# ihmcrobotics/mecano

Hardware: AMD Instinct MI355X
Metric: robot-configs/sec (RNEA+ABA), 30-DoF humanoid batch=4096 (higher is better)
Workload: dtype f64; 1 GPU; 30-DoF humanoid (SixDoF pelvis + 24 revolute), RNEA and ABA of every configuration per step, fp64, AoS [B][n] state; entry_point=mh_rnea_aba_f64, batch_per_gpu=4096, global_batch=4096, nq=31, nv=30, bodies=25, parallelism=dp1 (batch sharded, no data-path collective), kernel_variant=topo:b5c1e26c784c54fa, model_seed=43, state_seed=2342

## Files before the change

mecano_amd/csrc/mh_zv_kernels.h:

```cpp
#pragma once
#include "mh_spec_kernels.h"

namespace mh
{
template <class TP>
struct ZvStore
{
   static constexpr int REG_SLOTS = Split<TP>::zv_reg_slots();
   static constexpr int kind(int j) { return Split<TP>::is_trunk(j) ? ST_LDS_KIND : ST_REG_KIND; }
   static constexpr int index(int j) { return Split<TP>::is_trunk(j) ? Split<TP>::zv_trunk_slot(j) : Split<TP>::zv_reg_slot(j); }
   static constexpr bool shared(int j) { return !Split<TP>::is_trunk(j); }
};
template <class TP>
struct ZvbStore
{
   using S = Split<TP>;
   static constexpr bool root_in_regs(int j) { return S::staged() && j == S::root(); }
   static constexpr int REG_SLOTS = S::zv_reg_slots() + (S::staged() ? Tree<TP>::zv_slots_of(S::root() < 0 ? 0 : S::root(), true) : 0);
   static constexpr int trunk_slot(int j)
   {
      int s = 0;
      for (int i = 0; i < j; i++)
         s += S::is_trunk(i) && !root_in_regs(i) ? Tree<TP>::zv_slots_of(i, false) : 0;
      return s;
   }
   static constexpr int TRUNK_SLOTS = trunk_slot(TP::N);
   static constexpr int kind(int j) { return S::is_trunk(j) && !root_in_regs(j) ? ST_LDS_KIND : ST_REG_KIND; }
   static constexpr int index(int j) { return root_in_regs(j) ? S::zv_reg_slots() : (S::is_trunk(j) ? trunk_slot(j) : S::zv_reg_slot(j)); }
   static constexpr bool shared(int j) { return kind(j) == ST_REG_KIND; }
};
template <class TP>
struct ZvfPlan;
template <class TP>
struct ZvfStore
{
   using S = Split<TP>;
   using TR = Tree<TP>;
   static constexpr bool slot_homes = true;
   static constexpr bool mailed(int j) { return ZvfPlan<TP>::use_mail() && !S::is_trunk(j) && S::limb_index_of_body(j) == S::mailed_limb(); }
   static constexpr int slot_kind(int j, int k) { return mailed(j) && k >= 7 ? ST_LDS_KIND : kind(j); }
   static constexpr int slot_index(int j, int k) { return mailed(j) && k >= 7 ? ZvfPlan<TP>::mail_base() + (k - 7) : index(j) + k; }
   static constexpr bool root_in_regs(int j) { return S::staged() && j == S::root(); }
   static constexpr int limb_slots(int j) { return TR::zv_slots_of(j, true) + TR::ndof(j); }
   static constexpr int reg_slot(int j)
   {
      int s = 0;
      for (int i = 0; i < j; i++)
         s += !S::is_trunk(i) && S::owner(S::limb_index_of_body(i)) == S::owner(S::limb_index_of_body(j)) ? limb_slots(i) : 0;
      return s;
   }
   static constexpr int limb_reg_slots()
   {
      int best = 0;
      for (int w = 0; w < 4; w++)
      {
         int n = 0;
         for (int j = 0; j < TP::N; j++)
            n += !S::is_trunk(j) && S::owner(S::limb_index_of_body(j)) == w ? limb_slots(j) : 0;
         best = n > best ? n : best;
      }
      return best;
   }
   static constexpr int REG_SLOTS = limb_reg_slots() + (S::staged() ? TR::zv_slots_of(S::root() < 0 ? 0 : S::root(), true) : 0);
   static constexpr int trunk_slot(int j)
   {
      int s = 0;
      for (int i = 0; i < j; i++)
         s += S::is_trunk(i) && !root_in_regs(i) ? TR::zv_slots_of(i, false) + TR::ndof(i) : 0;
      return s;
   }
   static constexpr int root_tau_slot() { return trunk_slot(TP::N); }
   static constexpr int ROOT_TAU_SLOTS = S::staged() ? TR::ndof(S::root() < 0 ? 0 : S::root()) : 0;
   static constexpr bool owns_late(int w)
   {
      for (int k = 0; k < S::n_limbs(); k++)
         if (S::is_late(k) && S::owner(k) == w)
            return true;
      return false;
   }
   static constexpr bool late_body(int j) { return S::staged() && !S::is_trunk(j) && owns_late(S::owner(S::limb_index_of_body(j))); }
   static constexpr int late_tau_slot(int j)
   {
      int s = trunk_slot(TP::N) + ROOT_TAU_SLOTS;
      for (int i = 0; i < j; i++)
         s += late_body(i) ? TR::ndof(i) : 0;
      return s;
   }
   static constexpr int TRUNK_SLOTS = late_tau_slot(TP::N);
   static constexpr int tau_slot(int j) { return TR::zv_slots_of(j, !S::is_trunk(j)); }
   static constexpr int kind(int j) { return S::is_trunk(j) && !root_in_regs(j) ? ST_LDS_KIND : ST_REG_KIND; }
   static constexpr int index(int j) { return root_in_regs(j) ? limb_reg_slots() : (S::is_trunk(j) ? trunk_slot(j) : reg_slot(j)); }
   static constexpr bool shared(int j) { return kind(j) == ST_REG_KIND; }
};
#ifdef MH_ZV_PROBE
__device__ unsigned long long zv_probe[4096 * 3 * 4 * 16];
#define ZV_STAMP(job, ph)                                                                                                                  \
   do                                                                                                                                      \
   {                                                                                                                                       \
      const unsigned long long t_ = __builtin_amdgcn_s_memrealtime();                                                                      \
      if ((threadIdx.x & 63) == 0 && k < 4096)                                                                                             \
         zv_probe[((k * 3 + (job)) * 4 + (threadIdx.x >> 6)) * 16 + (ph)] = t_;                                                            \
   } while (0)
__device__ unsigned long long zv_probe_body[4096 * 32 * 4];
#ifdef MH_ZV_PROBE_BODY
#define ZV_STAMP_BODY(body, ph)                                                                                                            \
   do                                                                                                                                      \
   {                                                                                                                                       \
      const unsigned long long t_ = __builtin_amdgcn_s_memrealtime();                                                                      \
      if ((threadIdx.x & 63) == 0 && cx.own < 4096 && ((body) != 0 || cx.wave == 0))                                                      \
         zv_probe_body[(cx.own * 32 + (body)) * 4 + (ph)] = t_;                                                                            \
   } while (0)
#else
#define ZV_STAMP_BODY(body, ph)
#endif
#else
#define ZV_STAMP(job, ph)
#define ZV_STAMP_BODY(body, ph)
#endif
MH_DEV void zv_lds_barrier()
{
   asm volatile("s_waitcnt lgkmcnt(0)\n\ts_barrier" ::: "memory");
}
template <class CX>
MH_DEV void zv_fold_barrier()
{
   zv_lds_barrier();
}
constexpr int ZV_XW = 21;

template <int LIMB, class CX, typename T>
MH_DEV void x_put_ia(const CX &cx, const ABI<T> &I)
{
   constexpr int XW = ZV_XW;
   x_put<LIMB, XW, 0, CX, T>(cx, I.A.xx), x_put<LIMB, XW, 1, CX, T>(cx, I.A.xy), x_put<LIMB, XW, 2, CX, T>(cx, I.A.xz);
   x_put<LIMB, XW, 3, CX, T>(cx, I.A.yy), x_put<LIMB, XW, 4, CX, T>(cx, I.A.yz), x_put<LIMB, XW, 5, CX, T>(cx, I.A.zz);
   x_put<LIMB, XW, 6, CX, T>(cx, I.L.xx), x_put<LIMB, XW, 7, CX, T>(cx, I.L.xy), x_put<LIMB, XW, 8, CX, T>(cx, I.L.xz);
   x_put<LIMB, XW, 9, CX, T>(cx, I.L.yy), x_put<LIMB, XW, 10, CX, T>(cx, I.L.yz), x_put<LIMB, XW, 11, CX, T>(cx, I.L.zz);
   x_put<LIMB, XW, 12, CX, T>(cx, I.C.xx), x_put<LIMB, XW, 13, CX, T>(cx, I.C.xy), x_put<LIMB, XW, 14, CX, T>(cx, I.C.xz);
   x_put<LIMB, XW, 15, CX, T>(cx, I.C.yx), x_put<LIMB, XW, 16, CX, T>(cx, I.C.yy), x_put<LIMB, XW, 17, CX, T>(cx, I.C.yz);
   x_put<LIMB, XW, 18, CX, T>(cx, I.C.zx), x_put<LIMB, XW, 19, CX, T>(cx, I.C.zy), x_put<LIMB, XW, 20, CX, T>(cx, I.C.zz);
}
template <int LIMB, class CX, typename T>
MH_DEV ABI<T> x_get_ia(const CX &cx)
{
   constexpr int XW = ZV_XW;
   ABI<T> I;
   I.A = S3<T>{x_get<LIMB, XW, 0, CX, T>(cx), x_get<LIMB, XW, 1, CX, T>(cx), x_get<LIMB, XW, 2, CX, T>(cx),
               x_get<LIMB, XW, 3, CX, T>(cx), x_get<LIMB, XW, 4, CX, T>(cx), x_get<LIMB, XW, 5, CX, T>(cx)};
   I.L = S3<T>{x_get<LIMB, XW, 6, CX, T>(cx), x_get<LIMB, XW, 7, CX, T>(cx), x_get<LIMB, XW, 8, CX, T>(cx),
               x_get<LIMB, XW, 9, CX, T>(cx), x_get<LIMB, XW, 10, CX, T>(cx), x_get<LIMB, XW, 11, CX, T>(cx)};
   I.C = M3<T>{x_get<LIMB, XW, 12, CX, T>(cx), x_get<LIMB, XW, 13, CX, T>(cx), x_get<LIMB, XW, 14, CX, T>(cx),
               x_get<LIMB, XW, 15, CX, T>(cx), x_get<LIMB, XW, 16, CX, T>(cx), x_get<LIMB, XW, 17, CX, T>(cx),
               x_get<LIMB, XW, 18, CX, T>(cx), x_get<LIMB, XW, 19, CX, T>(cx), x_get<LIMB, XW, 20, CX, T>(cx)};
   return I;
}
template <typename T>
MH_DEV ABI<T> abi_zero()
{
   ABI<T> z;
   z.A = S3<T>{T(0), T(0), T(0), T(0), T(0), T(0)};
   z.L = z.A;
   z.C = M3<T>{T(0), T(0), T(0), T(0), T(0), T(0), T(0), T(0), T(0)};
   return z;
}
template <int J, int K0, class CX, typename T>
MH_DEV void st_put_ldl(const CX &cx, const LDL6<T> &F)
{
   cx.st.template put<J, 0>(F.f[0]), cx.st.template put<J, 1>(F.f[1]), cx.st.template put<J, 2>(F.f[2]), cx.st.template put<J, 3>(F.f[3]);
   cx.st.template put<J, 4>(F.f[4]), cx.st.template put<J, 5>(F.f[5]), cx.st.template put<J, 6>(F.f[6]), cx.st.template put<J, 7>(F.f[7]);
   cx.st.template put<J, 8>(F.f[8]), cx.st.template put<J, 9>(F.f[9]), cx.st.template put<J, 10>(F.f[10]), cx.st.template put<J, 11>(F.f[11]);
   cx.st.template put<J, 12>(F.f[12]), cx.st.template put<J, 13>(F.f[13]), cx.st.template put<J, 14>(F.f[14]), cx.st.template put<J, 15>(F.f[15]);
   cx.st.template put<J, 16>(F.f[16]), cx.st.template put<J, 17>(F.f[17]), cx.st.template put<J, 18>(F.f[18]), cx.st.template put<J, 19>(F.f[19]);
   cx.st.template put<J, 20>(F.f[20]);
}
template <int J, class CX, typename T>
MH_DEV LDL6<T> st_get_ldl(const CX &cx)
{
   LDL6<T> F;
   F.f[0] = cx.st.template get<J, 0>(), F.f[1] = cx.st.template get<J, 1>(), F.f[2] = cx.st.template get<J, 2>(), F.f[3] = cx.st.template get<J, 3>();
   F.f[4] = cx.st.template get<J, 4>(), F.f[5] = cx.st.template get<J, 5>(), F.f[6] = cx.st.template get<J, 6>(), F.f[7] = cx.st.template get<J, 7>();
   F.f[8] = cx.st.template get<J, 8>(), F.f[9] = cx.st.template get<J, 9>(), F.f[10] = cx.st.template get<J, 10>(), F.f[11] = cx.st.template get<J, 11>();
   F.f[12] = cx.st.template get<J, 12>(), F.f[13] = cx.st.template get<J, 13>(), F.f[14] = cx.st.template get<J, 14>(), F.f[15] = cx.st.template get<J, 15>();
   F.f[16] = cx.st.template get<J, 16>(), F.f[17] = cx.st.template get<J, 17>(), F.f[18] = cx.st.template get<J, 18>(), F.f[19] = cx.st.template get<J, 19>();
   F.f[20] = cx.st.template get<J, 20>();
   return F;
}

template <class TP, int J, class CX, typename T>
MH_DEV JX<T> zv_revolute_joint(const CX &cx)
{
   if constexpr (CX::csmode == 2)
   {
      constexpr int R = Tree<TP>::rev_index(J);
      JX<T> jx;
      jx.c = cx.cs[(2 * R) * cx.cs_stride], jx.s = cx.cs[(2 * R + 1) * cx.cs_stride], jx.d = T(0);
      return jx;
   }
   else
      return spec_joint<JT_REVOLUTE, Tree<TP>::cfg_ofs(J), CX, T>(cx);
}
template <class TP, int J, typename T, class CX, bool FAST = false>
struct ZvPre
{
   template <int K>
   static MH_DEV void children(const CX &cx, bool &bad)
   {
      if constexpr (K < Tree<TP>::n_children(J))
      {
         ZvPre<TP, Tree<TP>::child(J, K), T, CX, FAST>::run(cx, bad);
         children<K + 1>(cx, bad);
      }
   }
   static MH_DEV void run(const CX &cx, bool &bad)
   {
      children<0>(cx, bad);
      if constexpr (TP::type[J] == JT_REVOLUTE)
      {
         if constexpr (FAST && CX::csmode != 2)
         {
            const T x = cx.q(Tree<TP>::cfg_ofs(J));
            T s, c;
            sincos_fast(x, s, c);
            bad = bad || !sincos_in_fast_range(x);
            cx.st.template put<J, 7>(c);
            cx.st.template put<J, 8>(s);
         }
         else
         {
            const JX<T> jx = zv_revolute_joint<TP, J, CX, T>(cx);
            cx.st.template put<J, 7>(jx.c);
            cx.st.template put<J, 8>(jx.s);
         }
      }
   }
};
#ifndef MH_ZV_PRE_FAST
#define MH_ZV_PRE_FAST 1
#endif
template <class TP, int J, typename T, class CX>
MH_DEV void zv_pre(const CX &cx)
{
   bool bad = !MH_ZV_PRE_FAST;
   ZvPre<TP, J, T, CX, MH_ZV_PRE_FAST != 0>::run(cx, bad);
   if (__builtin_expect(bad, 0))
      ZvPre<TP, J, T, CX, false>::run(cx, bad);
}
template <class TP, int J, typename T, class CX, bool FAST = false>
struct ZvPreTrunk
{
   template <int K>
   static MH_DEV void children(const CX &cx, bool &bad)
   {
      if constexpr (K < Tree<TP>::n_children(J))
      {
         if constexpr (Split<TP>::is_trunk(Tree<TP>::child(J, K)))
            ZvPreTrunk<TP, Tree<TP>::child(J, K), T, CX, FAST>::run(cx, bad);
         children<K + 1>(cx, bad);
      }
   }
   static MH_DEV void run(const CX &cx, bool &bad)
   {
      children<0>(cx, bad);
      if constexpr (TP::type[J] == JT_REVOLUTE)
      {
         if constexpr (FAST && CX::csmode != 2)
         {
            const T x = cx.q(Tree<TP>::cfg_ofs(J));
            T s, c;
            sincos_fast(x, s, c);
            bad = bad || !sincos_in_fast_range(x);
// ... 40 lines not shown
   using S = Split<TP>;
   bool bad = false;
   zv_pre_limbs_of<TP, W, 0, T, CX, true>(cx, bad);
   if constexpr (S::staged())
      zv_pre_subtrunks_of<TP, W, 0, T, CX, true>(cx, bad);
   if (__builtin_expect(bad, 0))
   {
      zv_pre_limbs_of<TP, W, 0, T, CX, false>(cx, bad);
      if constexpr (S::staged())
         zv_pre_subtrunks_of<TP, W, 0, T, CX, false>(cx, bad);
   }
}
template <class TP, int J, typename T, class CX, int MODE = 0>
struct ZvIn
{
   template <int K>
   static MH_DEV void children(const CX &cx, ABI<T> &acc)
   {
      if constexpr (K < Tree<TP>::n_children(J))
      {
         constexpr int C = Tree<TP>::child(J, K);
         ABI<T> c;
         if constexpr ((MODE == 1 || MODE == 2) && !Split<TP>::is_trunk(C))
            c = x_get_ia<Split<TP>::limb_index(C), CX, T>(cx);
         else if constexpr (MODE == 2)
            c = x_get_ia<Split<TP>::sub_slot(C), CX, T>(cx);
         else
            c = ZvIn<TP, C, T, CX, MODE>::run(cx);
         if constexpr (K == 0)
            acc = c;
         else
            add(acc, c);
         children<K + 1>(cx, acc);
      }
   }
   static MH_DEV ABI<T> run(const CX &cx)
   {
      MH_BODY_FENCE();
      constexpr int TYPE = TP::type[J];
      constexpr bool HAS_PARENT = TP::parent[J] >= 0;
      constexpr bool LEAF = Tree<TP>::n_children(J) == 0;
      constexpr int CO = Tree<TP>::cfg_ofs(J);
      ABI<T> up = abi_zero<T>();
      if constexpr (!LEAF)
         children<0>(cx, up);
      if constexpr (MODE == 3 && Split<TP>::is_cut(J))
         __syncthreads();
      MH_BODY_FENCE();
      ZV_STAMP_BODY(J, 0);
      const T *cp = cx.C + J * MC_STRIDE;
      asm volatile("" : "+s"(cp));
      const CRef<T> c{cp};
      constexpr bool PRE = TYPE == JT_REVOLUTE && ((!Split<TP>::is_trunk(J) && (MODE == 0 || MODE == 3)) || ((CX::csmode == 2 || (CX::csmode == 0 && MH_ZV_PRE_WAVE)) && Split<TP>::staged() && Split<TP>::is_trunk(J) && MODE == 1) || (CX::csmode == 3 && Split<TP>::is_trunk(J)));
      JQ<T> jq;
      JX<T> jx;
      if constexpr (TYPE == JT_REVOLUTE && CX::csmode == 2 && !PRE)
         jx = zv_revolute_joint<TP, J, CX, T>(cx);
      else if constexpr (!PRE)
         jq = spec_joint_read<TYPE, CO, CX, T>(cx);
      const RI<T> I = load_inertia<T>(c);
      MH_BODY_FENCE();
      ABI<T> IA = abi_from_rigid(I);
      if constexpr (!LEAF)
         add(IA, up);
      MH_BODY_FENCE();
      ZV_STAMP_BODY(J, 1);
      const XF<T> Xb = load_xb_j<TP, J, T>(c);
      if constexpr (PRE)
         jx.c = cx.st.template get<J, 7>(), jx.s = cx.st.template get<J, 8>(), jx.d = T(0);
      else if constexpr (!(TYPE == JT_REVOLUTE && CX::csmode == 2))
         jx = spec_joint_from<TYPE, T>(jq);
      ABI<T> out = abi_zero<T>();
      if constexpr (TYPE == JT_REVOLUTE || TYPE == JT_PRISMATIC)
      {
         V3<T> ua, ul;
         T D;
         if constexpr (TYPE == JT_REVOLUTE)
            ua = V3<T>{IA.A.xz, IA.A.yz, IA.A.zz}, ul = V3<T>{IA.C.zx, IA.C.zy, IA.C.zz}, D = IA.A.zz;
         else
            ua = V3<T>{IA.C.xz, IA.C.yz, IA.C.zz}, ul = V3<T>{IA.L.xz, IA.L.yz, IA.L.zz}, D = IA.L.zz;
         const T dinv = rcp_fast(D);
         const V3<T> sa = dinv * ua, sl = dinv * ul;
         cx.st.template put<J, 0>(sa.x), cx.st.template put<J, 1>(sa.y), cx.st.template put<J, 2>(sa.z);
         cx.st.template put<J, 3>(sl.x), cx.st.template put<J, 4>(sl.y), cx.st.template put<J, 5>(sl.z);
         cx.st.template put<J, 6>(dinv);
         if constexpr (TYPE == JT_REVOLUTE)
         {
            cx.st.template put<J, 7>(jx.c);
            cx.st.template put<J, 8>(jx.s);
         }
         if constexpr (HAS_PARENT)
         {
            if constexpr (TYPE == JT_REVOLUTE)
               rank1_down_revolute(IA, ua, ul, dinv);
            else
               rank1_down(IA, ua, ul, dinv);
#ifdef MH_ZV_PROBE_BODY
            MH_BODY_FENCE();
            ZV_STAMP_BODY(J, 2);
#endif
            abi_up(TYPE, jx, Xb, IA);
            out = IA;
         }
      }
      else if constexpr (TYPE == JT_SIXDOF)
         st_put_ldl<J, 0, CX, T>(cx, spd6_factor(IA));
      else if constexpr (HAS_PARENT)
      {
         abi_up(TYPE, jx, Xb, IA);
         out = IA;
      }
      MH_BODY_FENCE();
      ZV_STAMP_BODY(J, 3);
      return out;
   }
};

template <class TP, int J, typename T, class CX, int MODE = 0>
struct ZvFold
{
   template <int K>
   static MH_DEV void children(const CX &cx, SV<T> &pA)
   {
      if constexpr (K < Tree<TP>::n_children(J))
      {
         constexpr int C = Tree<TP>::child(J, K);
         SV<T> c;
         if constexpr ((MODE == 1 || MODE == 2) && !Split<TP>::is_trunk(C))
            c = x_get6<Split<TP>::limb_index(C), CX::fold_xw, 0, CX, T>(cx);
         else if constexpr (MODE == 2)
            c = x_get6<Split<TP>::sub_slot(C), CX::fold_xw, 6, CX, T>(cx);
         else
            c = ZvFold<TP, C, T, CX, MODE>::run(cx);
         if constexpr (K == 0)
            pA = c;
         else
            pA = pA + c;
         children<K + 1>(cx, pA);
      }
   }
   static MH_DEV SV<T> run(const CX &cx)
   {
      MH_BODY_FENCE();
      constexpr int TYPE = TP::type[J];
      constexpr bool HAS_PARENT = TP::parent[J] >= 0;
      constexpr bool LEAF = Tree<TP>::n_children(J) == 0;
      constexpr int DO = Tree<TP>::dof_ofs(J), CO = Tree<TP>::cfg_ofs(J);
      constexpr int RS = Tree<TP>::zv_result_slot(J, CX::SPolicy::shared(J));
      const V3<T> Z{T(0), T(0), T(0)};
      SV<T> pA{Z, Z};
      if constexpr (!LEAF)
         children<0>(cx, pA);
      MH_BODY_FENCE();
      const T *cp = cx.C + J * MC_STRIDE;
      asm volatile("" : "+s"(cp));
      const CRef<T> c{cp};
      SV<T> up{Z, Z};
      if constexpr (TYPE == JT_REVOLUTE || TYPE == JT_PRISMATIC)
      {
         T tau;
         if constexpr (CX::csmode == 3)
            tau = zvf_tau_get1<TP, J, 0, CX, T>(cx);
         else
            tau = cx.in3(DO);
         JX<T> jx;
         jx.c = T(1), jx.s = T(0), jx.d = T(0);
         if constexpr (TYPE == JT_REVOLUTE)
            jx.c = cx.st.template get<J, 7>(), jx.s = cx.st.template get<J, 8>();
         else if constexpr (HAS_PARENT)
            jx.d = cx.q(CO);
         const V3<T> sa{cx.st.template get<J, 0>(), cx.st.template get<J, 1>(), cx.st.template get<J, 2>()};
         const V3<T> sl{cx.st.template get<J, 3>(), cx.st.template get<J, 4>(), cx.st.template get<J, 5>()};
         const T dinv = cx.st.template get<J, 6>();
         const T u = tau - (TYPE == JT_REVOLUTE ? pA.a.z : pA.l.z);
         cx.st.template put<J, RS>(u * dinv);
         if constexpr (HAS_PARENT)
         {
            const XF<T> Xb = load_xb_j<TP, J, T>(c);
            const SV<T> pa = pA + SV<T>{u * sa, u * sl};
            up = force_up(TYPE, jx, Xb, pa);
         }
      }
      else if constexpr (TYPE == JT_SIXDOF)
      {
         SV<T> tau;
         if constexpr (CX::csmode == 3)
            tau = SV<T>{V3<T>{zvf_tau_get1<TP, J, 0, CX, T>(cx), zvf_tau_get1<TP, J, 1, CX, T>(cx), zvf_tau_get1<TP, J, 2, CX, T>(cx)},
                        V3<T>{zvf_tau_get1<TP, J, 3, CX, T>(cx), zvf_tau_get1<TP, J, 4, CX, T>(cx), zvf_tau_get1<TP, J, 5, CX, T>(cx)}};
         else
            tau = spec_vec<TYPE, DO, 1, CX, T>(cx, true);
         const SV<T> x = spd6_solve(st_get_ldl<J, CX, T>(cx), tau - pA);
         cx.st.template put<J, RS + 0>(x.a.x), cx.st.template put<J, RS + 1>(x.a.y), cx.st.template put<J, RS + 2>(x.a.z);
         cx.st.template put<J, RS + 3>(x.l.x), cx.st.template put<J, RS + 4>(x.l.y), cx.st.template put<J, RS + 5>(x.l.z);
         if constexpr (HAS_PARENT)
         {
            const JX<T> jx = spec_joint<TYPE, CO, CX, T>(cx);
            up = force_up(TYPE, jx, load_xb_j<TP, J, T>(c), tau);
         }
      }
      else if constexpr (HAS_PARENT)
      {
         JX<T> jx;
         jx.c = T(1), jx.s = T(0), jx.d = T(0);
         up = force_up(TYPE, jx, load_xb_j<TP, J, T>(c), pA);
      }
      MH_BODY_FENCE();
      return up;
   }
};

template <class TP, int J, typename T, class CX, int MODE = 0>
struct ZvOut
{
   template <int K>
   static MH_DEV void children(const CX &cx, const SV<T> &a)
   {
      if constexpr (K < Tree<TP>::n_children(J))
      {
         constexpr int C = Tree<TP>::child(J, K);
         if constexpr (MODE == 1 && !Split<TP>::is_trunk(C))
         {
            if (cx.wave == Split<TP>::owner(Split<TP>::limb_index(C)))
               ZvOut<TP, C, T, CX, 0>::run(cx, a);
         }
         else
            ZvOut<TP, C, T, CX, MODE>::run(cx, a);
         children<K + 1>(cx, a);
      }
   }
   static MH_DEV void run(const CX &cx, const SV<T> &ap)
   {
      MH_BODY_FENCE();
      constexpr int TYPE = TP::type[J];
      constexpr bool HAS_PARENT = TP::parent[J] >= 0;
      constexpr bool LEAF = Tree<TP>::n_children(J) == 0;
      constexpr int DO = Tree<TP>::dof_ofs(J), CO = Tree<TP>::cfg_ofs(J);
      constexpr int RS = Tree<TP>::zv_result_slot(J, CX::SPolicy::shared(J));
      const T *cp = cx.C + J * MC_STRIDE;
      asm volatile("" : "+s"(cp));
      const CRef<T> c{cp};
      const V3<T> Z{T(0), T(0), T(0)};
      SV<T> a{Z, Z};
      if constexpr (HAS_PARENT)
      {
         JX<T> jx;
         jx.c = T(1), jx.s = T(0), jx.d = T(0);
         if constexpr (TYPE == JT_REVOLUTE)
            jx.c = cx.st.template get<J, 7>(), jx.s = cx.st.template get<J, 8>();
         else if constexpr (TYPE != JT_FIXED)
            jx = spec_joint<TYPE, CO, CX, T>(cx);
         a = motion_down(TYPE, jx, load_xb_j<TP, J, T>(c), ap);
      }
      if constexpr (TYPE == JT_REVOLUTE || TYPE == JT_PRISMATIC)
      {
         const V3<T> sa{cx.st.template get<J, 0>(), cx.st.template get<J, 1>(), cx.st.template get<J, 2>()};
         const V3<T> sl{cx.st.template get<J, 3>(), cx.st.template get<J, 4>(), cx.st.template get<J, 5>()};
         const T qdd = cx.st.template get<J, RS>() - (dot(sa, a.a) + dot(sl, a.l));
         if (MODE == 0 || cx.wave == 0)
            cx.out(DO, qdd);
         if constexpr (TYPE == JT_REVOLUTE)
            a.a.z += qdd;
         else
            a.l.z += qdd;
      }
      else if constexpr (TYPE == JT_SIXDOF)
      {
         const SV<T> x{V3<T>{cx.st.template get<J, RS + 0>(), cx.st.template get<J, RS + 1>(), cx.st.template get<J, RS + 2>()},
                       V3<T>{cx.st.template get<J, RS + 3>(), cx.st.template get<J, RS + 4>(), cx.st.template get<J, RS + 5>()}};
         if (MODE == 0 || cx.wave == 0)
            spec_write<TYPE, DO, CX, T>(cx, x - a);
         a = x;
      }
      MH_BODY_FENCE();
      if constexpr (!LEAF)
         children<0>(cx, a);
   }
};

template <class TP, typename T, class CX, int MODE, int K = 0>
MH_DEV void zv_roots_in(const CX &cx)
{
   if constexpr (K < Tree<TP>::n_children(-1))
   {
      (void)ZvIn<TP, Tree<TP>::child(-1, K), T, CX, MODE>::run(cx);
      zv_roots_in<TP, T, CX, MODE, K + 1>(cx);
   }
}
template <class TP, typename T, class CX, int K = 0>
MH_DEV void zv_roots_fold(const CX &cx)
{
   if constexpr (K < Tree<TP>::n_children(-1))
   {
      (void)ZvFold<TP, Tree<TP>::child(-1, K), T, CX, 1>::run(cx);
      zv_roots_fold<TP, T, CX, K + 1>(cx);
   }
}
template <class TP, typename T, class CX, int K = 0>
MH_DEV void zv_roots_out(const CX &cx)
{
   if constexpr (K < Tree<TP>::n_children(-1))
   {
      const V3<T> Z{T(0), T(0), T(0)};
      ZvOut<TP, Tree<TP>::child(-1, K), T, CX, 1>::run(cx, SV<T>{Z, Z});
      zv_roots_out<TP, T, CX, K + 1>(cx);
   }
}
template <class TP, int W, int K, int LATE, typename T, class CX>
MH_DEV void zv_limbs_in_of(const CX &cx)
{
   using S = Split<TP>;
   if constexpr (K < S::n_limbs())
   {
      if constexpr (S::owner(K) == W && (LATE < 0 || (S::is_late(K) ? 1 : 0) == LATE))
      {
         if constexpr (CX::csmode != 3 && !(CX::csmode == 0 && MH_ZV_PRE_WAVE))
            zv_pre<TP, S::limb_root(K), T, CX>(cx);
         x_put_ia<K, CX, T>(cx, ZvIn<TP, S::limb_root(K), T, CX, (LATE >= 0 && S::cut_limb(W) == K ? 3 : 0)>::run(cx));
      }
      zv_limbs_in_of<TP, W, K + 1, LATE, T, CX>(cx);
   }
}
template <class TP, int W, int I, typename T, class CX>
MH_DEV void zv_subtrunks_of(const CX &cx)
{
   using S = Split<TP>;
   if constexpr (I < S::n_sub())
   {
      constexpr int ST = S::sub_top(I);
      if constexpr (S::sub_owner(ST) == W)
         x_put_ia<S::sub_slot(ST), CX, T>(cx, ZvIn<TP, ST, T, CX, 1>::run(cx));
      zv_subtrunks_of<TP, W, I + 1, T, CX>(cx);
   }
}
template <class TP, int W, int J, typename T, class CX>
MH_DEV void zvf_park_late_tau(const CX &cx)
{
   using SP = typename CX::SPolicy;
   if constexpr (J < TP::N)
   {
      if constexpr (SP::late_body(J) && Split<TP>::owner(Split<TP>::limb_index_of_body(J)) == W)
      {
         constexpr int TS = SP::tau_slot(J), L0 = SP::late_tau_slot(J);
         cx.st.lbase[L0 * 64] = cx.st.template get<J, TS>();
         if constexpr (Tree<TP>::ndof(J) == 6)
         {
            cx.st.lbase[(L0 + 1) * 64] = cx.st.template get<J, TS + 1>(), cx.st.lbase[(L0 + 2) * 64] = cx.st.template get<J, TS + 2>();
            cx.st.lbase[(L0 + 3) * 64] = cx.st.template get<J, TS + 3>(), cx.st.lbase[(L0 + 4) * 64] = cx.st.template get<J, TS + 4>();
            cx.st.lbase[(L0 + 5) * 64] = cx.st.template get<J, TS + 5>();
         }
      }
      zvf_park_late_tau<TP, W, J + 1, T, CX>(cx);
   }
}
template <class TP, int W, typename T, class CX>
MH_DEV void zv_limbs_in(const CX &cx)
{
   using S = Split<TP>;
   if constexpr (W < 4)
   {
      if (cx.wave == W)
      {
         if constexpr (CX::csmode == 3)
            zvf_park_late_tau<TP, W, 0, T, CX>(cx);
         if constexpr (CX::csmode == 0 && MH_ZV_PRE_WAVE)
            zv_pre_wave<TP, W, T, CX>(cx);
         if constexpr (S::staged())
         {
            if constexpr (CX::csmode == 2)
            {
               bool unused = false;
               zv_pre_subtrunks_of<TP, W, 0, T, CX>(cx, unused);
            }
            zv_limbs_in_of<TP, W, 0, 0, T, CX>(cx);
            if constexpr (S::cut_limb(W) < 0)
               __syncthreads();
            zv_limbs_in_of<TP, W, 0, 1, T, CX>(cx);
            zv_subtrunks_of<TP, W, 0, T, CX>(cx);
         }
         else
            zv_limbs_in_of<TP, W, 0, -1, T, CX>(cx);
      }
      else
         zv_limbs_in<TP, W + 1, T, CX>(cx);
   }
}
template <class TP, int W, int K, typename T, class CX>
MH_DEV void zv_limbs_fold_of(const CX &cx)
{
   using S = Split<TP>;
   if constexpr (K < S::n_limbs())
   {
      if constexpr (S::owner(K) == W)
         x_put6<K, CX::fold_xw, 0, CX, T>(cx, ZvFold<TP, S::limb_root(K), T, CX, 0>::run(cx));
      zv_limbs_fold_of<TP, W, K + 1, T, CX>(cx);
   }
}
template <class TP, int W, typename T, class CX>
MH_DEV void zv_limbs_fold(const CX &cx)
{
   if constexpr (W < 4)
   {
      if (cx.wave == W)
         zv_limbs_fold_of<TP, W, 0, T, CX>(cx);
      else
         zv_limbs_fold<TP, W + 1, T, CX>(cx);
   }
}

template <class TP>
struct ZvWalk
{
   using S = Split<TP>;
   static constexpr bool below(int j, int top)
   {
      for (int a = j; a >= 0; a = TP::parent[a])
         if (a == top)
            return true;
      return false;
   }
   static constexpr bool needs(int W, int J)
   {
      for (int k = 0; k < S::n_limbs(); k++)
         if (S::owner(k) == W && below(S::limb_root(k), J))
            return true;
      return false;
   }
   static constexpr int writer(int J)
   {
      for (int w = 0; w < 4; w++)
         if (needs(w, J))
            return w;
      return 0;
   }
};
template <class TP, int J, int W, typename T, class CX>
struct ZvOutW
{
   template <int K>
   static MH_DEV void children(const CX &cx, const SV<T> &a)
   {
      if constexpr (K < Tree<TP>::n_children(J))
      {
         constexpr int C = Tree<TP>::child(J, K);
         if constexpr (!Split<TP>::is_trunk(C))
         {
            if constexpr (Split<TP>::owner(Split<TP>::limb_index(C)) == W)
               ZvOut<TP, C, T, CX, 0>::run(cx, a);
         }
         else if constexpr (ZvWalk<TP>::needs(W, C))
            ZvOutW<TP, C, W, T, CX>::run(cx, a);
         children<K + 1>(cx, a);
      }
   }
   static MH_DEV void run(const CX &cx, const SV<T> &ap)
   {
      MH_BODY_FENCE();
      constexpr int TYPE = TP::type[J];
      constexpr bool HAS_PARENT = TP::parent[J] >= 0;
      constexpr int DO = Tree<TP>::dof_ofs(J), CO = Tree<TP>::cfg_ofs(J);
      constexpr int RS = Tree<TP>::zv_result_slot(J, CX::SPolicy::shared(J));
      constexpr bool WRITES = ZvWalk<TP>::writer(J) == W;
      const T *cp = cx.C + J * MC_STRIDE;
      asm volatile("" : "+s"(cp));
      const CRef<T> c{cp};
      const V3<T> Z{T(0), T(0), T(0)};
      SV<T> a{Z, Z};
      if constexpr (HAS_PARENT)
      {
         JX<T> jx;
         jx.c = T(1), jx.s = T(0), jx.d = T(0);
         if constexpr (TYPE == JT_REVOLUTE)
            jx.c = cx.st.template get<J, 7>(), jx.s = cx.st.template get<J, 8>();
         else if constexpr (TYPE != JT_FIXED)
            jx = spec_joint<TYPE, CO, CX, T>(cx);
         a = motion_down(TYPE, jx, load_xb_j<TP, J, T>(c), ap);
      }
      if constexpr (TYPE == JT_REVOLUTE || TYPE == JT_PRISMATIC)
      {
         const V3<T> sa{cx.st.template get<J, 0>(), cx.st.template get<J, 1>(), cx.st.template get<J, 2>()};
         const V3<T> sl{cx.st.template get<J, 3>(), cx.st.template get<J, 4>(), cx.st.template get<J, 5>()};
         const T qdd = cx.st.template get<J, RS>() - (dot(sa, a.a) + dot(sl, a.l));
         if constexpr (WRITES)
            cx.out(DO, qdd);
         if constexpr (TYPE == JT_REVOLUTE)
            a.a.z += qdd;
         else
            a.l.z += qdd;
      }
      else if constexpr (TYPE == JT_SIXDOF)
      {
         const SV<T> x{V3<T>{cx.st.template get<J, RS + 0>(), cx.st.template get<J, RS + 1>(), cx.st.template get<J, RS + 2>()},
                       V3<T>{cx.st.template get<J, RS + 3>(), cx.st.template get<J, RS + 4>(), cx.st.template get<J, RS + 5>()}};
         if constexpr (WRITES)
            spec_write<TYPE, DO, CX, T>(cx, x - a);
         a = x;
      }
      MH_BODY_FENCE();
      children<0>(cx, a);
   }
};
template <class TP, int W, typename T, class CX, int K = 0>
MH_DEV void zv_roots_out_wave(const CX &cx)
{
   if constexpr (K < Tree<TP>::n_children(-1))
   {
      const V3<T> Z{T(0), T(0), T(0)};
      constexpr int R = Tree<TP>::child(-1, K);
      if constexpr (ZvWalk<TP>::needs(W, R) || ZvWalk<TP>::writer(R) == W)
         ZvOutW<TP, R, W, T, CX>::run(cx, SV<T>{Z, Z});
      zv_roots_out_wave<TP, W, T, CX, K + 1>(cx);
   }
}
template <class TP, int W, int K, int LATE, typename T, class CX>
MH_DEV void zv_limbs_fold_sel(const CX &cx)
{
   using S = Split<TP>;
   if constexpr (K < S::n_limbs())
   {
      if constexpr (S::owner(K) == W && (LATE < 0 || (S::is_late(K) ? 1 : 0) == LATE))
         x_put6<K, CX::fold_xw, 0, CX, T>(cx, ZvFold<TP, S::limb_root(K), T, CX, 0>::run(cx));
      zv_limbs_fold_sel<TP, W, K + 1, LATE, T, CX>(cx);
   }
}
template <class TP, int W, int I, typename T, class CX>
MH_DEV void zv_subtrunks_fold_of(const CX &cx)
{
   using S = Split<TP>;
   if constexpr (I < S::n_sub())
   {
      constexpr int ST = S::sub_top(I);
      if constexpr (S::sub_owner(ST) == W)
         x_put6<S::sub_slot(ST), CX::fold_xw, 6, CX, T>(cx, ZvFold<TP, ST, T, CX, 1>::run(cx));
      zv_subtrunks_fold_of<TP, W, I + 1, T, CX>(cx);
   }
}
struct ZvNoHook
{
   MH_DEV void after_early() const {}
   MH_DEV void after_late() const {}
   MH_DEV void before_out() const {}
};
template <class TP, int W, typename T, class CX, class HOOK = ZvNoHook>
MH_DEV void zv_fold_out(const CX &cx, const HOOK &hook = HOOK())
{
   using S = Split<TP>;
   if constexpr (W < 4)
   {
      if (cx.wave == W)
      {
         if constexpr (S::staged())
         {
#ifdef MH_ZV_PROBE
            const long k = (long)cx.own;
#endif
            zv_limbs_fold_sel<TP, W, 0, 0, T, CX>(cx);
            hook.after_early();
            ZV_STAMP(1, 7);
            zv_fold_barrier<CX>();
            zv_limbs_fold_sel<TP, W, 0, 1, T, CX>(cx);
            hook.after_late();
            zv_subtrunks_fold_of<TP, W, 0, T, CX>(cx);
            ZV_STAMP(1, 8);
            zv_fold_barrier<CX>();
            (void)ZvFold<TP, S::root(), T, CX, 2>::run(cx);
            ZV_STAMP(1, 9);
         }
         else
         {
            zv_limbs_fold_sel<TP, W, 0, -1, T, CX>(cx);
            hook.after_early();
            zv_fold_barrier<CX>();
            hook.after_late();
            zv_roots_fold<TP, T, CX>(cx);
         }
         if constexpr (CX::csmode >= 2)
            zv_fold_barrier<CX>();
         hook.before_out();
         asm volatile("" ::: "memory");
         zv_roots_out_wave<TP, W, T, CX>(cx);
      }
      else
         zv_fold_out<TP, W + 1, T, CX, HOOK>(cx, hook);
   }
}

template <typename T, int N, int NT>
MH_DEV void zv_stage_rows(lds_ptr<T> dst, const T *src, int rows)
{
   constexpr int U = (64 * N + NT - 1) / NT;
   T r[U];
   const int n = rows * N, t = threadIdx.x;
#pragma unroll
   for (int u = 0; u < U; u++)
      r[u] = t + NT * u < n ? src[t + NT * u] : T(0);
#pragma unroll
   for (int u = 0; u < U; u++)
      if (t + NT * u < 64 * N)
         dst[t + NT * u] = r[u];
}

struct ZvSync
{
   int *flags;
   int *error;
   int epoch;
   int jobs;
   int same_l2;
   unsigned wait_ticks;
};
MH_DEV int zv_xcc_id() { return (int)(__builtin_amdgcn_s_getreg((31 << 11) | 20) & 0xf); }
MH_DEV int zv_mail_key(int epoch, int xcc) { return (int)(((unsigned)epoch & 0x03ffffffu) << 5) | 16 | xcc; }

MH_DEV bool zv_wait(const ZvSync &sy, long k)
{
   const int *f = sy.flags + k * ZV_SYNC_STRIDE;
   if (__hip_atomic_load(f, __ATOMIC_RELAXED, __HIP_MEMORY_SCOPE_AGENT) == sy.epoch)
      return true;
   const unsigned long long t0 = __builtin_amdgcn_s_memrealtime();
   for (;;)
   {
      __builtin_amdgcn_s_sleep(1);
      if (__hip_atomic_load(f, __ATOMIC_RELAXED, __HIP_MEMORY_SCOPE_AGENT) == sy.epoch)
         return true;
      if (__builtin_amdgcn_s_memrealtime() - t0 > (unsigned long long)sy.wait_ticks)
      {
         if ((threadIdx.x & 63) == 0)
            __hip_atomic_store(sy.error, 1, __ATOMIC_RELAXED, __HIP_MEMORY_SCOPE_SYSTEM);
         return false;
      }
   }
}
template <typename T, int NT>
MH_DEV void zv_publish_rows(T *dst, lds_ptr<T> src, int n, bool same_l2)
{
   if (same_l2)
      for (int i = threadIdx.x; i < n; i += NT)
         __hip_atomic_store(dst + i, src[i], __ATOMIC_RELAXED, __HIP_MEMORY_SCOPE_WORKGROUP);
   else
      for (int i = threadIdx.x; i < n; i += NT)
         __hip_atomic_store(dst + i, src[i], __ATOMIC_RELAXED, __HIP_MEMORY_SCOPE_AGENT);
}
template <typename T, int N, int NT>
MH_DEV void zv_fetch_rows(lds_ptr<T> dst, const T *src, int rows)
{
   constexpr int U = (64 * N + NT - 1) / NT;
   T r[U];
   const int n = rows * N, t = threadIdx.x;
#pragma unroll
   for (int u = 0; u < U; u++)
      r[u] = t + NT * u < n ? __hip_atomic_load(src + t + NT * u, __ATOMIC_RELAXED, __HIP_MEMORY_SCOPE_AGENT) : T(0);
#pragma unroll
   for (int u = 0; u < U; u++)
      if (t + NT * u < 64 * N)
         dst[t + NT * u] = r[u];
}

template <typename T, int N, int NT>
struct RowRegs
{
   static constexpr int U = (64 * N + NT - 1) / NT;
   T r[U];
   MH_DEV void issue(const T *src, int rows, int t = threadIdx.x)
   {
      const int last = rows * N - 1;
#pragma unroll
      for (int u = 0; u < U; u++)
         r[u] = src[t + NT * u < last ? t + NT * u : last];
   }
   MH_DEV void commit(lds_ptr<T> dst, int t = threadIdx.x) const
   {
#pragma unroll
      for (int u = 0; u < U; u++)
         if (t + NT * u < 64 * N)
            dst[t + NT * u] = r[u];
   }
};
#ifndef MH_ZV_TWO_STAGE
#define MH_ZV_TWO_STAGE 1
#endif
template <class TP>
struct ZvCols
{
   static constexpr int NV = Tree<TP>::total_dofs();
   static constexpr int body_of(int d)
   {
      for (int j = 0; j < TP::N; j++)
         if (d >= Tree<TP>::dof_ofs(j) && d < Tree<TP>::dof_ofs(j) + Tree<TP>::ndof(j))
            return j;
      return 0;
   }
   static constexpr bool trunk(int d) { return Split<TP>::is_trunk(body_of(d)); }
   static constexpr int aba_owner(int d) { return trunk(d) ? -1 : Split<TP>::owner(Split<TP>::limb_index_of_body(body_of(d))); }
   static constexpr int limb_number(int d)
   {
      int n = 0;
      for (int c = 0; c < d; c++)
         n += trunk(c) ? 0 : 1;
      return n;
   }
};
template <class TP, typename T, int OWNER>
struct ZvColRegs
{
   static constexpr int count()
   {
      int n = 0;
      for (int d = 0; d < ZvCols<TP>::NV; d++)
         n += ZvCols<TP>::aba_owner(d) == OWNER ? 1 : 0;
      return n;
   }
   T r[count() > 0 ? count() : 1];
   template <int D = 0, int K = 0>
   MH_DEV void issue(const T *src, int lane)
   {
      if constexpr (D < ZvCols<TP>::NV)
      {
         if constexpr (ZvCols<TP>::aba_owner(D) == OWNER)
         {
            r[K] = __hip_atomic_load(src + D * 64 + lane, __ATOMIC_RELAXED, __HIP_MEMORY_SCOPE_AGENT);
            issue<D + 1, K + 1>(src, lane);
         }
         else
            issue<D + 1, K>(src, lane);
      }
   }
   template <int D = 0, int K = 0>
   MH_DEV void commit(lds_ptr<T> row) const
   {
      if constexpr (D < ZvCols<TP>::NV)
      {
         if constexpr (ZvCols<TP>::aba_owner(D) == OWNER)
         {
// ... 286 lines not shown
   cx.st.gbase = nullptr, cx.st.stride = 0, cx.st.lane = 0;
   if (active)
      split_rnea_limbs<TP, 0, T, CX>(cx);
   ZV_STAMP(0, 2);
   if (threadIdx.x == 64)
      zv_same_l2 = sy.same_l2 && __hip_atomic_load(sy.flags + k * ZV_SYNC_STRIDE + 32, __ATOMIC_RELAXED, __HIP_MEMORY_SCOPE_AGENT) == zv_mail_key(sy.epoch, zv_xcc_id());
   __syncthreads();
   ZV_STAMP(0, 3);
   const bool same = zv_same_l2 != 0;
   if (active && wave == 0)
      rnea_trunk_roots<TP, T, CX>(cx);
   ZV_STAMP(0, 4);
   __syncthreads();
   zv_publish_rows<T, 256>(taup + cfg0 * nv, lx, rows * nv, same);
   ZV_STAMP(0, 5);
#ifdef MH_ZV_TEST_FLAG_BEFORE_DRAIN
   if (threadIdx.x == 0)
      __hip_atomic_store(sy.flags + k * ZV_SYNC_STRIDE, sy.epoch, __ATOMIC_RELAXED, __HIP_MEMORY_SCOPE_AGENT);
#endif
   asm volatile("s_waitcnt vmcnt(0)" ::: "memory");
   ZV_STAMP(0, 6);
   __syncthreads();
#if !defined(MH_ZV_TEST_FLAG_BEFORE_DRAIN) && !defined(MH_ZV_TEST_NO_FLAG)
   if (threadIdx.x == 0)
   {
      if (same)
         __hip_atomic_store(sy.flags + k * ZV_SYNC_STRIDE, sy.epoch, __ATOMIC_RELAXED, __HIP_MEMORY_SCOPE_WORKGROUP);
      else
         __hip_atomic_store(sy.flags + k * ZV_SYNC_STRIDE, sy.epoch, __ATOMIC_RELAXED, __HIP_MEMORY_SCOPE_AGENT);
   }
#endif
   ZV_STAMP(0, 7);
}

template <class TP, typename T, bool IDENT>
MH_DEV void zv_aba_group(const Args<T> &A, long k, lds_ptr<T> lds, const T *taup, const ZvSync &sy)
{
   using S = Split<TP>;
#ifndef MH_ZV_DIRECT_OUT
#define MH_ZV_DIRECT_OUT 0
#endif
   using CX = Ctx<T, true, IDENT, ZvStore<TP>, false, MH_ZV_DIRECT_OUT ? 2 : 0>;
   const int wave = __builtin_amdgcn_readfirstlane((int)(threadIdx.x >> 6));
   const int lane = threadIdx.x & 63;
   const int nq = A.m.nq, nv = A.m.nv;
   const lds_ptr<T> lxc = lds, lst = lxc + S::n_limbs() * ZV_XW * 64, lq = lst + S::ZV_TRUNK_SLOTS * 64, lx = lq + 64 * nq, lres = lx + 64 * nv;
   ZV_STAMP(1, 14);
   const long cfg0 = k * 64;
   const int rows = (int)(A.B - cfg0 < 64 ? A.B - cfg0 : 64);
   const bool active = lane < rows;
   ZV_STAMP(1, 0);
   if (sy.same_l2 && threadIdx.x == 0)
      __hip_atomic_store(sy.flags + k * ZV_SYNC_STRIDE + 32, zv_mail_key(sy.epoch, zv_xcc_id()), __ATOMIC_RELAXED, __HIP_MEMORY_SCOPE_AGENT);
   zv_stage_rows<T, Tree<TP>::total_cfgs(), 256>(lq, A.q + cfg0 * nq, rows);
   __syncthreads();
   ZV_STAMP(1, 1);
   CX cx;
   fill_ctx<T>(cx, A, active ? cfg0 + lane : cfg0);
   cx.lq = lq + lane * nq, cx.lqd = lq, cx.lx = lx + lane * nv, cx.lo = lres + lane * nv;
   cx.wave = wave;
   cx.xbase = lxc + lane;
   cx.st.lbase = lst + lane;
   cx.st.gbase = nullptr, cx.st.stride = 0, cx.st.lane = 0;
#ifdef MH_ZV_PROBE
   cx.own = (unsigned long long)k;
#endif
#ifdef MH_ZV_TWICE
#pragma unroll 1
   for (int rep = 0; rep < 2; rep++)
   {
      asm volatile("" ::: "memory");
      if (active)
         zv_limbs_in<TP, 0, T, CX>(cx);
      if (rep == 0)
      {
         ZV_STAMP(1, 12);
         __syncthreads();
         ZV_STAMP(1, 13);
      }
   }
#else
   if (active)
      zv_limbs_in<TP, 0, T, CX>(cx);
#endif
   ZV_STAMP(1, 2);
   __syncthreads();
   ZV_STAMP(1, 3);
   if (active)
      zv_roots_in<TP, T, CX, (S::staged() ? 2 : 1)>(cx);
   ZV_STAMP(1, 4);
   __shared__ int zv_gave_up;
   if (wave == 0)
   {
      const bool seen = zv_wait(sy, k);
      if (lane == 0)
         zv_gave_up = seen ? 0 : 1;
   }
   __syncthreads();
   if (zv_gave_up)
   {
      for (int i = threadIdx.x; i < rows * nv; i += 256)
      {
         if constexpr (sizeof(T) == 8)
            reinterpret_cast<unsigned long long *>(A.out)[cfg0 * nv + i] = 0x7ff8000000000000ull;
         else
            reinterpret_cast<unsigned *>(A.out)[cfg0 * nv + i] = 0x7fc00000u;
      }
      return;
   }
   ZV_STAMP(1, 5);
   zv_fetch_rows<T, Tree<TP>::total_dofs(), 256>(lx, taup + cfg0 * nv, rows);
   if (threadIdx.x == 0)
   {
      __hip_atomic_store(sy.flags + k * ZV_SYNC_STRIDE, 0, __ATOMIC_RELAXED, __HIP_MEMORY_SCOPE_AGENT);
      if (sy.same_l2)
         __hip_atomic_store(sy.flags + k * ZV_SYNC_STRIDE + 32, 0, __ATOMIC_RELAXED, __HIP_MEMORY_SCOPE_AGENT);
   }
   __syncthreads();
   ZV_STAMP(1, 6);
   asm volatile("" ::: "memory");
   if (active)
      zv_fold_out<TP, 0, T, CX>(cx);
   ZV_STAMP(1, 10);
   if constexpr (!MH_ZV_DIRECT_OUT)
   {
      __syncthreads();
      wave_copy_out<T, 256>(A.out + cfg0 * nv, lres, rows * nv);
   }
   ZV_STAMP(1, 11);
}

MH_DEV bool zv_wait_word(const ZvSync &sy, const int *f)
{
   if (__hip_atomic_load(f, __ATOMIC_RELAXED, __HIP_MEMORY_SCOPE_AGENT) == sy.epoch)
      return true;
   const unsigned long long t0 = __builtin_amdgcn_s_memrealtime();
   for (;;)
   {
      __builtin_amdgcn_s_sleep(1);
      if (__hip_atomic_load(f, __ATOMIC_RELAXED, __HIP_MEMORY_SCOPE_AGENT) == sy.epoch)
         return true;
      if (__builtin_amdgcn_s_memrealtime() - t0 > (unsigned long long)sy.wait_ticks)
      {
         if ((threadIdx.x & 63) == 0)
            __hip_atomic_store(sy.error, 1, __ATOMIC_RELAXED, __HIP_MEMORY_SCOPE_SYSTEM);
         return false;
      }
   }
}
template <class TP, typename T, bool STEP>
MH_DEV void zv_aba_group2(const Args<T> &A, long k, lds_ptr<T> lds, const T *taup, const ZvSync &sy)
{
   using S = Split<TP>;
   using CX = Ctx<T, true, true, ZvStore<TP>, false, 0>;
   const int wave = __builtin_amdgcn_readfirstlane((int)(threadIdx.x >> 6));
   const int lane = threadIdx.x & 63;
   constexpr int nq = Tree<TP>::total_cfgs(), nv = Tree<TP>::total_dofs();
   const lds_ptr<T> lxc = lds, lst = lxc + S::n_limbs() * ZV_XW * 64, lq = lst + S::ZV_TRUNK_SLOTS * 64, lx = lq + 64 * nq, lres = lx + 64 * nv;
   ZV_STAMP(1, 14);
   const long cfg0 = k * 64;
   const int rows = (int)(A.B - cfg0 < 64 ? A.B - cfg0 : 64);
   const bool active = lane < rows;
   __shared__ int zv_gave_up;
   if (threadIdx.x == 0)
      zv_gave_up = 0;
   ZV_STAMP(1, 0);
#if MH_ZV_SELF_SIGNAL
   const int poison = __hip_atomic_load(sy.flags + ZV_POISON_WORD, __ATOMIC_RELAXED, __HIP_MEMORY_SCOPE_AGENT);
#endif
   zv_stage_rows<T, Tree<TP>::total_cfgs(), 256>(lq, A.q + cfg0 * nq, rows);
   __syncthreads();
   ZV_STAMP(1, 1);
   CX cx;
   fill_ctx<T>(cx, A, active ? cfg0 + lane : cfg0);
   cx.lq = lq + lane * nq, cx.lqd = lq, cx.lx = lx + lane * nv, cx.lo = lres + lane * nv;
   cx.wave = wave;
   cx.xbase = lxc + lane;
   cx.st.lbase = lst + lane;
   cx.st.gbase = nullptr, cx.st.stride = 0, cx.st.lane = 0;
#ifdef MH_ZV_PROBE
   cx.own = (unsigned long long)k;
#endif
   if (active)
      zv_limbs_in<TP, 0, T, CX>(cx);
   ZV_STAMP(1, 2);
   __syncthreads();
   ZV_STAMP(1, 3);
   if (active)
      zv_roots_in<TP, T, CX, (S::staged() ? 2 : 1)>(cx);
   ZV_STAMP(1, 4);
   RowRegs<T, STEP ? Tree<TP>::total_dofs() : 1, 256> rqd;
   if constexpr (STEP)
      rqd.issue(A.qd + cfg0 * nv, rows);
   const T *const src = taup + k * 64 * nv;
   const int *const flags = sy.flags + k * ZV_SYNC_STRIDE;
   const lds_ptr<T> row = lx + lane * nv;
#if MH_ZV_SELF_SIGNAL
   bool seen;
   {
      T *const back = const_cast<T *>(src);
      if (wave == 0)
         seen = zv_take_cols<TP, T, 0>(sy, src, back, row, lane, active, poison);
      else if (wave == 1)
         seen = zv_take_cols<TP, T, 1>(sy, src, back, row, lane, active, poison);
      else if (wave == 2)
         seen = zv_take_cols<TP, T, 2>(sy, src, back, row, lane, active, poison);
      else
         seen = zv_take_cols<TP, T, 3>(sy, src, back, row, lane, active, poison);
   }
   ZV_STAMP(1, 5);
#else
   bool seen = zv_wait_word(sy, flags + 1);
   ZV_STAMP(1, 5);
   if (wave == 0)
   {
      ZvColRegs<TP, T, 0> c;
      c.issue(src, lane), c.commit(row);
   }
   else if (wave == 1)
   {
      ZvColRegs<TP, T, 1> c;
      c.issue(src, lane), c.commit(row);
   }
   else if (wave == 2)
   {
      ZvColRegs<TP, T, 2> c;
      c.issue(src, lane), c.commit(row);
   }
   else
   {
      ZvColRegs<TP, T, 3> c;
      c.issue(src, lane), c.commit(row);
   }
#endif
   const int b_first = __hip_atomic_load(flags, __ATOMIC_RELAXED, __HIP_MEMORY_SCOPE_AGENT);
   zv_lds_barrier();
   ZV_STAMP(1, 6);
   asm volatile("" ::: "memory");
   struct TrunkTau : ZvNoHook
   {
      mutable ZvColRegs<TP, T, -1> c;
      const ZvSync &sy;
      const int *flags;
      const T *src;
      lds_ptr<T> row;
      int lane, b_first;
      bool &seen;
      MH_DEV void after_early() const
      {
         if (b_first != sy.epoch)
            seen = zv_wait_word(sy, flags) && seen;
         c.issue(src, lane);
      }
      MH_DEV void after_late() const { c.commit(row); }
   };
   const TrunkTau trunk{{}, {}, sy, flags, src, row, lane, b_first, seen};
   if (active)
      zv_fold_out<TP, 0, T, CX>(cx, trunk);
   ZV_STAMP(1, 10);
   if (!seen && lane == 0)
      zv_gave_up = 1;
   __syncthreads();
   if (threadIdx.x == 0)
   {
      __hip_atomic_store(const_cast<int *>(flags), 0, __ATOMIC_RELAXED, __HIP_MEMORY_SCOPE_AGENT);
      __hip_atomic_store(const_cast<int *>(flags) + 1, 0, __ATOMIC_RELAXED, __HIP_MEMORY_SCOPE_AGENT);
   }
   if (zv_gave_up)
   {
      for (int i = threadIdx.x; i < rows * nv; i += 256)
         reinterpret_cast<unsigned long long *>(A.out)[cfg0 * nv + i] = 0x7ff8000000000000ull;
      if constexpr (STEP)
      {
         for (int i = threadIdx.x; i < rows * nq; i += 256)
            reinterpret_cast<unsigned long long *>(A.q_next)[cfg0 * nq + i] = 0x7ff8000000000000ull;
         for (int i = threadIdx.x; i < rows * nv; i += 256)
            reinterpret_cast<unsigned long long *>(A.qd_next)[cfg0 * nv + i] = 0x7ff8000000000000ull;
      }
      return;
   }
   if constexpr (STEP)
   {
      rqd.commit(lx);
      __syncthreads();
      if (active)
         integrate_rows<TP, 0, T>(wave, lq + lane * nq, lx + lane * nv, lres + lane * nv, A.dt, T(0.5) * A.dt * A.dt);
      __syncthreads();
      wave_copy_out<T, 256>(A.q_next + cfg0 * nq, lq, rows * nq);
      wave_copy_out<T, 256>(A.qd_next + cfg0 * nv, lx, rows * nv);
   }
   wave_copy_out<T, 256>(A.out + cfg0 * nv, lres, rows * nv);
   ZV_STAMP(1, 11);
}

#ifndef MH_ZV_KERNEL_ATTR
#define MH_ZV_KERNEL_ATTR
#endif
template <class TP, typename T, bool IDENT, bool STEP = false>
__global__ void __launch_bounds__(256) MH_ZV_KERNEL_ATTR spec_zv_kernel(const T *q0, const T *qd0, const T *tau0, long B0, int jobs0, Args<T> A_full, T *taup,
                                                                        ZvSync sy_full)
{
   extern __shared__ double lds_raw[];
   const int blk = (int)blockIdx.x;
   Args<T> A = A_full;
   A.q = q0, A.qd = qd0, A.in3b = tau0, A.B = B0;
   ZvSync sy = sy_full;
   sy.jobs = jobs0;
// ... 468 lines not shown
```

Measured before the change: 305.5 million configs/s.

## Relay trunk accelerations to late-limb owners via LDS flags in ABA outward pass

Adds a relay mode to the ABA outward pass. A wave that does not own late limbs posts the parent trunk acceleration for early limbs of a busy wave into LDS and raises a per-limb flag. The owning wave then spin-waits on that flag instead of redundantly walking the trunk path itself. The aim is to cut duplicated trunk recomputation in the tail, at the cost of an intra-workgroup LDS handshake and polling. It also adds optional tail timing stamps behind a probe macro.

```diff
diff --git a/mecano_amd/csrc/mh_zv_kernels.h b/mecano_amd/csrc/mh_zv_kernels.h
--- a/mecano_amd/csrc/mh_zv_kernels.h
+++ b/mecano_amd/csrc/mh_zv_kernels.h
@@ -113,9 +113,21 @@
 #else
 #define ZV_STAMP_BODY(body, ph)
 #endif
+#ifdef MH_ZV_PROBE_TAIL
+#define ZV_STAMP_TAIL(body, ph)                                                                                                            \
+   do                                                                                                                                      \
+   {                                                                                                                                       \
+      const unsigned long long t_ = __builtin_amdgcn_s_memrealtime();                                                                      \
+      if ((threadIdx.x & 63) == 0 && cx.own < 4096 && ((body) != 0 || cx.wave == 0))                                                      \
+         zv_probe_body[(cx.own * 32 + (body)) * 4 + (ph)] = t_;                                                                            \
+   } while (0)
+#else
+#define ZV_STAMP_TAIL(body, ph)
+#endif
 #else
 #define ZV_STAMP(job, ph)
 #define ZV_STAMP_BODY(body, ph)
+#define ZV_STAMP_TAIL(body, ph)
 #endif
 MH_DEV void zv_lds_barrier()
 {
@@ -462,6 +474,7 @@
       if constexpr (!LEAF)
          children<0>(cx, pA);
       MH_BODY_FENCE();
+      ZV_STAMP_TAIL(J, 0);
       const T *cp = cx.C + J * MC_STRIDE;
       asm volatile("" : "+s"(cp));
       const CRef<T> c{cp};
@@ -515,6 +528,7 @@
          up = force_up(TYPE, jx, load_xb_j<TP, J, T>(c), pA);
       }
       MH_BODY_FENCE();
+      ZV_STAMP_TAIL(J, 1);
       return up;
    }
 };
@@ -546,6 +560,7 @@
       constexpr bool LEAF = Tree<TP>::n_children(J) == 0;
       constexpr int DO = Tree<TP>::dof_ofs(J), CO = Tree<TP>::cfg_ofs(J);
       constexpr int RS = Tree<TP>::zv_result_slot(J, CX::SPolicy::shared(J));
+      ZV_STAMP_TAIL(J, 2);
       const T *cp = cx.C + J * MC_STRIDE;
       asm volatile("" : "+s"(cp));
       const CRef<T> c{cp};
@@ -582,6 +597,7 @@
          a = x;
       }
       MH_BODY_FENCE();
+      ZV_STAMP_TAIL(J, 3);
       if constexpr (!LEAF)
          children<0>(cx, a);
    }
@@ -717,7 +733,22 @@
    }
 }
 
-template <class TP>
+template <class CXB>
+struct ZvRelayCtx : CXB
+{
+   static constexpr bool relay = true;
+};
+template <class CX, class = void>
+struct zv_relay
+{
+   static constexpr bool value = false;
+};
+template <class CX>
+struct zv_relay<CX, std::enable_if_t<CX::relay>>
+{
+   static constexpr bool value = true;
+};
+template <class TP, bool RELAY = false>
 struct ZvWalk
 {
    using S = Split<TP>;
@@ -728,10 +759,27 @@
             return true;
       return false;
    }
+   static constexpr bool owns_late(int W)
+   {
+      for (int k = 0; k < S::n_limbs(); k++)
+         if (S::owner(k) == W && S::is_late(k))
+            return true;
+      return false;
+   }
+   static constexpr int poster(int k)
+   {
+      if (!RELAY || !S::staged() || S::is_late(k) || !owns_late(S::owner(k)) || TP::parent[S::limb_root(k)] == S::root())
+         return -1;
+      for (int w = 0; w < 4; w++)
+         if (!owns_late(w) && ZvWalk<TP, false>::needs(w, TP::parent[S::limb_root(k)]))
+            return w;
+      return -1;
+   }
+   static constexpr bool relayed(int k) { return poster(k) >= 0; }
    static constexpr bool needs(int W, int J)
    {
       for (int k = 0; k < S::n_limbs(); k++)
-         if (S::owner(k) == W && below(S::limb_root(k), J))
+         if (S::owner(k) == W && below(S::limb_root(k), J) && !relayed(k))
             return true;
       return false;
    }
@@ -743,9 +791,37 @@
       return 0;
    }
 };
+constexpr int ZV_RELAY_A = 12, ZV_RELAY_FLAG = 18;
+template <class TP, int J, int W, int K, typename T, class CX>
+MH_DEV void zv_relay_post(const CX &cx, const SV<T> &a)
+{
+   using S = Split<TP>;
+   if constexpr (K < S::n_limbs())
+   {
+      if constexpr (TP::parent[S::limb_root(K)] == J && ZvWalk<TP, true>::poster(K) == W)
+      {
+         x_put6<K, ZV_XW, ZV_RELAY_A, CX, T>(cx, a);
+         asm volatile("s_waitcnt lgkmcnt(0)" ::: "memory");
+         __hip_atomic_store(cx.xbase + (K * ZV_XW + ZV_RELAY_FLAG) * 64, T(1), __ATOMIC_RELAXED, __HIP_MEMORY_SCOPE_WORKGROUP);
+      }
+      zv_relay_post<TP, J, W, K + 1, T, CX>(cx, a);
+   }
+}
+template <class TP, int W, int K, typename T, class CX>
+MH_DEV void zv_relay_clear(const CX &cx)
+{
+   using S = Split<TP>;
+   if constexpr (K < S::n_limbs())
+   {
+      if constexpr (S::owner(K) == W && ZvWalk<TP, true>::relayed(K))
+         x_put<K, ZV_XW, ZV_RELAY_FLAG, CX, T>(cx, T(0));
+      zv_relay_clear<TP, W, K + 1, T, CX>(cx);
+   }
+}
 template <class TP, int J, int W, typename T, class CX>
 struct ZvOutW
 {
+   using WK = ZvWalk<TP, zv_relay<CX>::value>;
    template <int K>
    static MH_DEV void children(const CX &cx, const SV<T> &a)
    {
@@ -754,10 +830,10 @@
          constexpr int C = Tree<TP>::child(J, K);
          if constexpr (!Split<TP>::is_trunk(C))
          {
-            if constexpr (Split<TP>::owner(Split<TP>::limb_index(C)) == W)
+            if constexpr (Split<TP>::owner(Split<TP>::limb_index(C)) == W && !WK::relayed(Split<TP>::limb_index(C)))
                ZvOut<TP, C, T, CX, 0>::run(cx, a);
          }
-         else if constexpr (ZvWalk<TP>::needs(W, C))
+         else if constexpr (WK::needs(W, C))
             ZvOutW<TP, C, W, T, CX>::run(cx, a);
          children<K + 1>(cx, a);
       }
@@ -769,7 +845,9 @@
       constexpr bool HAS_PARENT = TP::parent[J] >= 0;
       constexpr int DO = Tree<TP>::dof_ofs(J), CO = Tree<TP>::cfg_ofs(J);
       constexpr int RS = Tree<TP>::zv_result_slot(J, CX::SPolicy::shared(J));
-      constexpr bool WRITES = ZvWalk<TP>::writer(J) == W;
+      constexpr bool WRITES = WK::writer(J) == W;
+      if constexpr (WRITES)
+         ZV_STAMP_TAIL(J, 2);
       const T *cp = cx.C + J * MC_STRIDE;
       asm volatile("" : "+s"(cp));
       const CRef<T> c{cp};
@@ -806,6 +884,10 @@
          a = x;
       }
       MH_BODY_FENCE();
+      if constexpr (WRITES)
+         ZV_STAMP_TAIL(J, 3);
+      if constexpr (zv_relay<CX>::value)
+         zv_relay_post<TP, J, W, 0, T, CX>(cx, a);
       children<0>(cx, a);
    }
 };
@@ -816,9 +898,27 @@
    {
       const V3<T> Z{T(0), T(0), T(0)};
       constexpr int R = Tree<TP>::child(-1, K);
-      if constexpr (ZvWalk<TP>::needs(W, R) || ZvWalk<TP>::writer(R) == W)
+      using WK = ZvWalk<TP, zv_relay<CX>::value>;
+      if constexpr (WK::needs(W, R) || WK::writer(R) == W)
          ZvOutW<TP, R, W, T, CX>::run(cx, SV<T>{Z, Z});
       zv_roots_out_wave<TP, W, T, CX, K + 1>(cx);
+   }
+}
+template <class TP, int W, int K, typename T, class CX>
+MH_DEV void zv_relay_out(const CX &cx)
+{
+   using S = Split<TP>;
+   if constexpr (K < S::n_limbs())
+   {
+      if constexpr (S::owner(K) == W && ZvWalk<TP, true>::relayed(K))
+      {
+         const lds_ptr<T> flag = cx.xbase + (K * ZV_XW + ZV_RELAY_FLAG) * 64;
+         while (__builtin_amdgcn_ballot_w64(__hip_atomic_load(flag, __ATOMIC_RELAXED, __HIP_MEMORY_SCOPE_WORKGROUP) == T(0)) != 0)
+            __builtin_amdgcn_s_sleep(1);
+         asm volatile("" ::: "memory");
+         ZvOut<TP, S::limb_root(K), T, CX, 0>::run(cx, x_get6<K, ZV_XW, ZV_RELAY_A, CX, T>(cx));
+      }
+      zv_relay_out<TP, W, K + 1, T, CX>(cx);
    }
 }
 template <class TP, int W, int K, int LATE, typename T, class CX>
@@ -863,6 +963,8 @@
 #ifdef MH_ZV_PROBE
             const long k = (long)cx.own;
 #endif
+            if constexpr (zv_relay<CX>::value)
+               zv_relay_clear<TP, W, 0, T, CX>(cx);
             zv_limbs_fold_sel<TP, W, 0, 0, T, CX>(cx);
             hook.after_early();
             ZV_STAMP(1, 7);
@@ -888,6 +990,8 @@
          hook.before_out();
          asm volatile("" ::: "memory");
          zv_roots_out_wave<TP, W, T, CX>(cx);
+         if constexpr (zv_relay<CX>::value)
+            zv_relay_out<TP, W, 0, T, CX>(cx);
       }
       else
          zv_fold_out<TP, W + 1, T, CX, HOOK>(cx, hook);
@@ -1480,7 +1584,7 @@
 MH_DEV void zv_aba_group2(const Args<T> &A, long k, lds_ptr<T> lds, const T *taup, const ZvSync &sy)
 {
    using S = Split<TP>;
-   using CX = Ctx<T, true, true, ZvStore<TP>, false, 0>;
+   using CX = ZvRelayCtx<Ctx<T, true, true, ZvStore<TP>, false, 0>>;
    const int wave = __builtin_amdgcn_readfirstlane((int)(threadIdx.x >> 6));
    const int lane = threadIdx.x & 63;
    constexpr int nq = Tree<TP>::total_cfgs(), nv = Tree<TP>::total_dofs();
```

Result: faster. 314.2 million configs/s (median of 6 runs) (+2.8%).
